# WPCLab/OpenSeg3D

Measured on AMD Instinct MI355X. Metric: points/sec fwd+bwd, Waymo 1-sweep ~180k pts @0.1m voxel; logit parity, higher is better.
Workload: dtype f32 storage/accumulate, bf16x3 products; 1 GPU; waymo_one_sweep (BASELINE configs[1]): synthetic scene, 174633 pts/step/GPU, voxel [0.1, 0.1, 0.1], grid [1440, 1440, 64], fwd (attention dropout p=0.1, DropPath) + criterion (ohem_ce+lovasz on 3 heads) + bwd + SGD step; mode=fwdbwd, segmentor=segformer, voxels=108690, parallelism=dp1

## Files before the change

include/seg3d_hip.h:

```cpp
#ifndef SEG3D_HIP_H
#define SEG3D_HIP_H

#include <stddef.h>
#include <stdint.h>

#ifdef __cplusplus
extern "C" {
#endif

#define SEG3D_OK 0
#define SEG3D_EINVAL (-1)
#define SEG3D_EWORKSPACE (-2)
#define SEG3D_ELAUNCH (-3)

#define SEG3D_REDUCE_SUM 0
#define SEG3D_REDUCE_MEAN 1
#define SEG3D_REDUCE_MAX 2

int seg3d_abi_version(void);

const char* seg3d_last_error(void);

int seg3d_grid_size(const float* voxel_size, const float* range, int32_t* grid_xyz);

// ... 324 lines not shown

#define SEG3D_CRITERION_MAX_HEADS 4
#define SEG3D_CRITERION_CE 1
#define SEG3D_CRITERION_LOVASZ 2
#define SEG3D_CRITERION_STATS_STRIDE 68
typedef struct {
    const float* logits;
    const int64_t* labels;
    int64_t n;
    float weight;
} seg3d_criterion_head;
typedef struct {
    int32_t n_heads;
    seg3d_criterion_head heads[SEG3D_CRITERION_MAX_HEADS];
} seg3d_criterion_table;
size_t seg3d_criterion_workspace_bytes(const seg3d_criterion_table* heads, int32_t c, int32_t terms);
int seg3d_criterion_fwd(const seg3d_criterion_table* heads, int32_t c, int32_t terms, int64_t ignore_index,
                        float keep_thresh, float w_ce, float w_lovasz, float* lse, float* coef, float* stats, float* loss,
                        void* workspace, size_t workspace_bytes, void* stream);
int seg3d_criterion_bwd(const seg3d_criterion_table* heads, int32_t c, int32_t terms, float w_ce, float w_lovasz,
                        const float* lse, const float* coef, const float* stats, const float* grad_out,
                        float* const* dlogits, void* stream);

size_t seg3d_pointwise_loss_workspace_bytes(int64_t n);
int seg3d_focal_loss_fwd(const float* logits, const int64_t* labels, int64_t n, int32_t c, int64_t ignore_index, float gamma,
                         float alpha, const float* class_weight, int32_t reduction, float* stats, void* workspace,
                         size_t workspace_bytes, void* stream);
int seg3d_focal_loss_bwd(const float* logits, const int64_t* labels, const float* stats, const float* grad_out, int64_t n,
                         int32_t c, int64_t ignore_index, float gamma, float alpha, const float* class_weight,
                         int32_t reduction, float* dlogits, void* stream);

int seg3d_dice_loss_fwd(const float* logits, const int64_t* labels, int64_t n, int32_t c, int64_t ignore_index, float smooth,
                        float exponent, const float* class_weight, float loss_weight, float avg_factor, float* loss,
                        void* workspace, size_t workspace_bytes, void* stream);
int seg3d_dice_loss_bwd(const float* logits, const int64_t* labels, const float* grad_out, int64_t n, int32_t c,
                        int64_t ignore_index, float smooth, float exponent, const float* class_weight, float loss_weight,
                        float avg_factor, float* dlogits, void* stream);

#define SEG3D_CE_SELECT_MEAN_WEIGHTED 0
#define SEG3D_CE_SELECT_MEAN_ALL 1
#define SEG3D_CE_SELECT_THRESH 2
#define SEG3D_CE_SELECT_RATIO 3
size_t seg3d_ce_select_workspace_bytes(int64_t n);
int seg3d_ce_select_fwd(const float* logits, const int64_t* labels, int64_t n, int32_t c, int64_t ignore_index,
                        const float* class_weight, int32_t mode, float keep_thresh, double keep_ratio, float* lse,
                        float* stats, void* workspace, size_t workspace_bytes, void* stream);
// ... 187 lines not shown
```

openseg3d_amd/_lib.py:

```python
import ctypes
import os
import re

_HERE = os.path.dirname(os.path.abspath(__file__))
LIB_PATH = os.path.join(_HERE, "csrc", "libseg3d_hip.so")
HEADER_PATH = os.path.join(os.path.dirname(_HERE), "include", "seg3d_hip.h")

OK, EINVAL, EWORKSPACE, ELAUNCH = 0, -1, -2, -3
REDUCE_SUM, REDUCE_MEAN, REDUCE_MAX = 0, 1, 2
ABI_VERSION = 53

_p, _i32, _i64, _sz, _f = ctypes.c_void_p, ctypes.c_int32, ctypes.c_int64, ctypes.c_size_t, ctypes.c_float
_u64 = ctypes.c_uint64
_d = ctypes.c_double

SIGNATURES = {
    "seg3d_abi_version": (ctypes.c_int, []),
    "seg3d_last_error": (ctypes.c_char_p, []),
    "seg3d_grid_size": (ctypes.c_int, [_p, _p, _p]),
    "seg3d_voxelize_workspace_bytes": (_sz, [_i64]),
    "seg3d_voxelize_f32": (ctypes.c_int, [_p, _i64, _i32, _i32, _i32, _p, _p, _p, _p, _p, _p, _sz, _p]),
    "seg3d_voxelize_f64": (ctypes.c_int, [_p, _i64, _i32, _i32, _i32, _p, _p, _p, _p, _p, _p, _sz, _p]),
    "seg3d_voxelize_host_workspace_bytes": (_sz, [_i64]),
    "seg3d_voxelize_host_f32": (ctypes.c_int, [_p, _i64, _i32, _i32, _i32, _p, _p, _p, _p, _p, _p, _sz]),
    "seg3d_voxelize_host_f64": (ctypes.c_int, [_p, _i64, _i32, _i32, _i32, _p, _p, _p, _p, _p, _p, _sz]),
    "seg3d_cart2polar_f32": (ctypes.c_int, [_p, _i64, _i32, _i32, _p, _p]),
    "seg3d_cart2polar_f64": (ctypes.c_int, [_p, _i64, _i32, _i32, _p, _p]),
    "seg3d_group_index_workspace_bytes": (_sz, [_i64, _i64]),
    "seg3d_group_index": (ctypes.c_int, [_p, _i64, _i64, _p, _p, _p, _p, _sz, _p]),
    "seg3d_coord_hash_bytes": (_sz, [_i64]),
    "seg3d_coord_hash_build": (ctypes.c_int, [_p, _i64, _p, _p, _sz, _p]),
    "seg3d_rulebook_subm": (ctypes.c_int, [_p, _i64, _p, _p, _sz, _p, _p]),
    "seg3d_downsample_workspace_bytes": (_sz, [_i32, _p]),
# ... 55 lines not shown
    "seg3d_layernorm_bwd_workspace_bytes": (ctypes.c_size_t, [_i64, _i32]),
    "seg3d_layernorm_bwd": (ctypes.c_int, [_p, _p, _p, _p, _p, _p, _i64, _i32, _p, _p, _p, _p, ctypes.c_size_t, _p]),
    "seg3d_layernorm_bwd_partials": (ctypes.c_int, [_p, _p, _p, _p, _p, _p, _i64, _i32, _p, _p, ctypes.c_size_t, _p, _p]),
    "seg3d_batchnorm_workspace_bytes": (ctypes.c_size_t, [_i64, _i32]),
    "seg3d_colstats": (ctypes.c_int, [_p, _i64, _i32, _p, _p, ctypes.c_size_t, _p]),
    "seg3d_batchnorm_stats": (ctypes.c_int, [_p, _i64, _i32, _f, _p, _p, _f, _p, _p, _p, _p, ctypes.c_size_t, _p]),
    "seg3d_affine_act": (ctypes.c_int, [_p, _p, _p, _p, _i32, _i64, _i32, _p, _p]),
    "seg3d_gelu_fwd": (ctypes.c_int, [_p, _i64, _p, _p, _p]),
    "seg3d_batchnorm_bwd": (ctypes.c_int, [_p, _p, _p, _p, _p, _p, _i32, _i64, _i32, _p, _p, _p, _p, ctypes.c_size_t, _p]),
    "seg3d_batchnorm_bwd_reduce": (ctypes.c_int, [_p, _p, _p, _p, _p, _i32, _i64, _i32, _p, _p, ctypes.c_size_t, _p]),
    "seg3d_batchnorm_bwd_apply": (ctypes.c_int, [_p, _p, _p, _p, _p, _p, _p, _p, _i32, _i64, _i32, _p, _p, _p]),
    "seg3d_segment_reduce_fwd": (ctypes.c_int, [_p, _i32, _p, _p, _i64, _i32, _p, _p, _p]),
    "seg3d_segment_reduce_bwd": (ctypes.c_int, [_p, _i32, _p, _i64, _p, _p, _i64, _i32, _p, _p]),
    "seg3d_voxel_majority_labels": (ctypes.c_int, [_p, _p, _p, _i64, _i32, _p, _p]),
    "seg3d_cross_entropy_workspace_bytes": (ctypes.c_size_t, [_i64]),
    "seg3d_cross_entropy_fwd": (ctypes.c_int, [_p, _p, _i64, _i32, _i64, _f, _p, _p, _p, ctypes.c_size_t, _p]),
    "seg3d_cross_entropy_bwd": (ctypes.c_int, [_p, _p, _p, _p, _p, _i64, _i32, _p, _p]),
    "seg3d_lovasz_workspace_bytes": (ctypes.c_size_t, [_i64, _i32]),
    "seg3d_lovasz_softmax_fwd": (ctypes.c_int, [_p, _p, _i64, _i32, _i64, _i32, _p, _p, _p, _p, _p, ctypes.c_size_t, _p]),
    "seg3d_lovasz_softmax_bwd": (ctypes.c_int, [_p, _p, _p, _p, _i64, _i32, _p, _p]),
    "seg3d_criterion_workspace_bytes": (ctypes.c_size_t, [_p, _i32, _i32]),
    "seg3d_criterion_fwd": (ctypes.c_int, [_p, _i32, _i32, _i64, _f, _f, _f, _p, _p, _p, _p, _p, ctypes.c_size_t, _p]),
    "seg3d_criterion_bwd": (ctypes.c_int, [_p, _i32, _i32, _f, _f, _p, _p, _p, _p, _p, _p]),
    "seg3d_pointwise_loss_workspace_bytes": (ctypes.c_size_t, [_i64]),
    "seg3d_focal_loss_fwd": (ctypes.c_int, [_p, _p, _i64, _i32, _i64, _f, _f, _p, _i32, _p, _p, ctypes.c_size_t, _p]),
    "seg3d_focal_loss_bwd": (ctypes.c_int, [_p, _p, _p, _p, _i64, _i32, _i64, _f, _f, _p, _i32, _p, _p]),
    "seg3d_dice_loss_fwd": (ctypes.c_int, [_p, _p, _i64, _i32, _i64, _f, _f, _p, _f, _f, _p, _p, ctypes.c_size_t, _p]),
    "seg3d_dice_loss_bwd": (ctypes.c_int, [_p, _p, _p, _i64, _i32, _i64, _f, _f, _p, _f, _f, _p, _p]),
    "seg3d_ce_select_workspace_bytes": (ctypes.c_size_t, [_i64]),
    "seg3d_ce_select_fwd": (ctypes.c_int, [_p, _p, _i64, _i32, _i64, _p, _i32, _f, ctypes.c_double, _p, _p, _p,
                                           ctypes.c_size_t, _p]),
    "seg3d_ce_select_bwd": (ctypes.c_int, [_p, _p, _p, _p, _p, _p, _i64, _i32, _i32, _p, _p]),
    "seg3d_knn_level_workspace_bytes": (ctypes.c_size_t, [_i64]),
    "seg3d_knn_level_build": (ctypes.c_int, [_p, _i64, _p, _i32, _f, _p, _p, _p, _p, _p, _i64, _p, ctypes.c_size_t, _p]),
    "seg3d_parity_order": (ctypes.c_int, [_p, _i64, _p, _p, ctypes.c_size_t, _p]),
    "seg3d_knn_query_order": (ctypes.c_int, [_p, _i64, _p, _i32, _f, _p, _p, ctypes.c_size_t, _p]),
    "seg3d_knn_grid_query": (ctypes.c_int, [_p, _i32, _p, _p, _i64, _p, _p, _i32, _i32, _p, _p, _p]),
    "seg3d_knn_query": (ctypes.c_int, [_p, _i64, _p, _i64, _p, _p, _i32, _i32, _p, _p, _p]),
    "seg3d_furthest_sampling_workspace_bytes": (_sz, [_i64]),
    "seg3d_furthest_sampling": (ctypes.c_int, [_p, _i64, _p, _p, _p, _i32, _p, _p, _sz, _p]),
    "seg3d_furthest_sampling_host": (ctypes.c_int, [_p, _i64, _p, _p, _p, _i32, _p]),
    "seg3d_sector_angles": (ctypes.c_int, [_p, _i64, _p, _i32, _p, _p, _p]),
    "seg3d_sector_angles_host": (ctypes.c_int, [_p, _i64, _p, _i32, _p, _p]),
    "seg3d_sector_assign": (ctypes.c_int, [_p, _i64, _p, _i32, _p, _p, _p, _p]),
    "seg3d_sector_assign_host": (ctypes.c_int, [_p, _i64, _p, _i32, _p, _p, _p]),
    "seg3d_pointops_scratch_bytes": (_sz, [_i64, _i32, _i32]),
# ... 116 lines not shown
```

openseg3d_amd/csrc/criterion.hip:

```cpp
#include <rocprim/device/device_radix_sort.hpp>

#include "criterion_device.hpp"

namespace {

using crit::class_bits;
using crit::kChunk;
using crit::kMaxBlocks;
using crit::kMaxClasses;
using crit::kThreads;
using Key = unsigned long long;

constexpr int kMaxHeads = SEG3D_CRITERION_MAX_HEADS;
constexpr int kErrBits = 30;
constexpr uint32_t kErrMask = (1u << kErrBits) - 1u;
constexpr int kStatsStride = SEG3D_CRITERION_STATS_STRIDE;

struct Head {
    const float* x;
    const int64_t* y;
    float* dx;
    int n;
    int row0;
    int blk0, nblk;
    int bblk0;
    int nchunks;
    int chunk0;
    int64_t sorted0;
    float weight;
};

struct Heads {
    int nh;
    Head h[kMaxHeads];
};

struct Plan {
    Heads hd;
    int64_t rows, total;
    int row_blocks, bwd_blocks, pairs;
    int sort_bits;
    size_t sort_bytes;
};

__device__ __forceinline__ int head_of(const Heads& hd, int idx, int Head::*first) {
    int h = 0;
    for (int i = 1; i < hd.nh; ++i)
        if (idx >= hd.h[i].*first) h = i;
    return h;
}

__global__ __launch_bounds__(kThreads) void criterion_rows_kernel(Heads hd, int c, int terms, int64_t ignore_index,
                                                                  float keep_thresh, float* __restrict__ lse,
                                                                  float* __restrict__ ce_part ,
                                                                  Key* __restrict__ keys, uint32_t* __restrict__ vals) {
    const int hi = head_of(hd, (int)blockIdx.x, &Head::blk0);
    const Head& H = hd.h[hi];
    const int n = H.n;
    const int64_t in0 = (int64_t)H.row0 * c;
    const int blk = (int)blockIdx.x - H.blk0;
    const float* __restrict__ x = H.x;
    const int64_t* __restrict__ label = H.y;
    float loss = 0.f, cnt = 0.f;
    for (int64_t r = (int64_t)blk * kThreads + threadIdx.x; r < n; r += (int64_t)H.nblk * kThreads) {
        const float* __restrict__ row = x + r * c;
        float m, s;
        crit::softmax_stats(row, c, &m, &s);
        const int64_t y = label[r];
        if (terms & SEG3D_CRITERION_CE) {
            float l;
            const bool counted = crit::ce_row(row, c, y, ignore_index, keep_thresh, m, s, &l);
            lse[H.row0 + r] = counted ? l : INFINITY;
            if (counted) {
                loss += l - row[y];
                cnt += 1.f;
            }
        }
        if (terms & SEG3D_CRITERION_LOVASZ) {
            const bool valid = y != ignore_index;
            for (int j = 0; j < c; ++j) {
                const bool fg = valid && y == j;
                const int64_t at = in0 + (int64_t)j * n + r;
                keys[at] = ((Key)(hi * c + j) << kErrBits) | (crit::lovasz_err_bits(row, j, m, s, valid, fg) & kErrMask);
                vals[at] = (uint32_t)(H.row0 + r) | (fg ? 0x80000000u : 0u);
            }
        }
    }
    if (terms & SEG3D_CRITERION_CE) {
        crit::block_sum2(loss, cnt);
        if (threadIdx.x == 0) {
            ce_part[2 * blockIdx.x] = loss;
            ce_part[2 * blockIdx.x + 1] = cnt;
        }
    }
}

__global__ __launch_bounds__(kThreads) void criterion_count_kernel(Heads hd, const uint32_t* __restrict__ vals,
                                                                   int* __restrict__ chunk_cnt) {
    const Head& H = hd.h[head_of(hd, (int)blockIdx.x, &Head::chunk0)];
    const int local = (int)blockIdx.x - H.chunk0;
    const int seg = local / H.nchunks, chunk = local - seg * H.nchunks;
    const int t = crit::lovasz_chunk_count(vals + H.sorted0 + (int64_t)seg * H.n, H.n, chunk);
    if (threadIdx.x == 0) chunk_cnt[blockIdx.x] = t;
}

__global__ __launch_bounds__(64) void criterion_offsets_kernel(Heads hd, int c, const int* __restrict__ chunk_cnt,
                                                               int* __restrict__ chunk_off, int* __restrict__ total) {
    const int hi = (int)blockIdx.x / c, seg = (int)blockIdx.x - hi * c;
    const Head& H = hd.h[hi];
    const int at = H.chunk0 + seg * H.nchunks;
    const int t = crit::lovasz_segment_offsets(chunk_cnt + at, H.nchunks, chunk_off + at);
    if (threadIdx.x == 0) total[blockIdx.x] = t;
}

__global__ __launch_bounds__(kThreads) void criterion_grad_kernel(Heads hd, int c, const Key* __restrict__ keys,
                                                                  const uint32_t* __restrict__ vals,
                                                                  const int* __restrict__ chunk_off,
                                                                  const int* __restrict__ total, float* __restrict__ coef,
                                                                  float* __restrict__ part) {
    const int hi = head_of(hd, (int)blockIdx.x, &Head::chunk0);
    const Head& H = hd.h[hi];
    const int local = (int)blockIdx.x - H.chunk0;
    const int seg = local / H.nchunks, chunk = local - seg * H.nchunks;
    const int64_t seg0 = H.sorted0 + (int64_t)seg * H.n;
    const float t = crit::lovasz_chunk_grad(keys + seg0, vals + seg0, kErrMask, H.n, c, c - 1 - seg, chunk,
                                            chunk_off[blockIdx.x], total[hi * c + seg], coef);
    if (threadIdx.x == 0) part[blockIdx.x] = t;
}

__global__ __launch_bounds__(kThreads) void criterion_finalize_kernel(Heads hd, int c, int terms, float w_ce, float w_lovasz,
                                                                      const float* __restrict__ ce_part,
                                                                      const float* __restrict__ part,
                                                                      const int* __restrict__ total,
                                                                      float* __restrict__ stats, float* __restrict__ out) {
    for (int hi = 0; hi < hd.nh; ++hi) {
        const Head& H = hd.h[hi];
        float* st = stats + hi * kStatsStride;
        if (terms & SEG3D_CRITERION_CE) {
            float mean, count;
            crit::ce_mean(ce_part + 2 * H.blk0, H.nblk, &mean, &count);
            if (threadIdx.x == 0) {
                st[0] = mean;
                st[1] = count;
            }
            __syncthreads();
        }
        if (terms & SEG3D_CRITERION_LOVASZ) {
// ... 89 lines not shown
    Heads& hd = pl->hd;
    hd.nh = nh;
    int row0 = 0, blk0 = 0, bblk0 = 0, chunk0 = 0;
    const int tile = bwd_tile_rows(c, terms);
    for (int i = 0; i < nh; ++i) {
        Head& H = hd.h[i];
        const int64_t n = tab->heads[i].n;
        H.x = tab->heads[i].logits;
        H.y = tab->heads[i].labels;
        H.dx = nullptr;
        H.n = (int)n;
        H.weight = tab->heads[i].weight;
        H.row0 = row0;
        H.blk0 = blk0;
        H.nblk = (int)(ceil_div64(n, kThreads) > kMaxBlocks ? kMaxBlocks : ceil_div64(n, kThreads));
        H.bblk0 = bblk0;
        H.nchunks = (int)ceil_div64(n, kChunk);
        H.chunk0 = chunk0;
        row0 += (int)n;
        blk0 += H.nblk;
        bblk0 += (int)ceil_div64(n, tile);
        chunk0 += c * H.nchunks;
    }
    int64_t behind = 0;
    for (int i = nh - 1; i >= 0; --i) {
        hd.h[i].sorted0 = behind;
        behind += (int64_t)hd.h[i].n * c;
    }
    pl->rows = rows;
    pl->total = rows * c;
    pl->row_blocks = blk0;
    pl->bwd_blocks = bblk0;
    pl->pairs = chunk0;
    pl->sort_bits = kErrBits + class_bits(nh * c);
    pl->sort_bytes = 0;
    return SEG3D_OK;
}

int plan_sort_scratch(int terms, Plan* pl) {
    if (!(terms & SEG3D_CRITERION_LOVASZ) || pl->total == 0) return SEG3D_OK;
    rocprim::double_buffer<Key> k(nullptr, nullptr);
    rocprim::double_buffer<uint32_t> v(nullptr, nullptr);
    size_t bytes = 0;
    if (rocprim::radix_sort_pairs_desc(nullptr, bytes, k, v, (size_t)pl->total, 0u, (unsigned)pl->sort_bits) != hipSuccess)
        return SEG3D_ELAUNCH;
    pl->sort_bytes = bytes;
    return SEG3D_OK;
}

size_t fixed_bytes(const Plan& pl, int c, int terms) {
    size_t b = align_up((size_t)(pl.row_blocks > 0 ? pl.row_blocks : 1) * 2 * sizeof(float), 256);
    if (terms & SEG3D_CRITERION_LOVASZ) {
        const size_t t = (size_t)pl.total, cc = (size_t)pl.pairs;
        b += 2 * align_up(t * sizeof(Key), 256) + 2 * align_up(t * sizeof(uint32_t), 256) + 2 * align_up(cc * sizeof(int), 256) +
             align_up(cc * sizeof(float), 256) + align_up((size_t)pl.hd.nh * c * sizeof(int), 256);
    }
    return b + 256;
}

}

extern "C" size_t seg3d_criterion_workspace_bytes(const seg3d_criterion_table* heads, int32_t c, int32_t terms) {
    Plan pl;
    if (make_plan(heads, c, terms, &pl) != SEG3D_OK || plan_sort_scratch(terms, &pl) != SEG3D_OK) return 0;
    return fixed_bytes(pl, c, terms) + align_up(pl.sort_bytes, 256);
}

extern "C" int seg3d_criterion_fwd(const seg3d_criterion_table* heads, int32_t c, int32_t terms, int64_t ignore_index,
                                   float keep_thresh, float w_ce, float w_lovasz, float* lse, float* coef, float* stats,
// ... 9 lines not shown
    if (workspace_bytes < fixed_bytes(pl, c, terms) + align_up(pl.sort_bytes, 256)) return SEG3D_EWORKSPACE;
    hipStream_t st = as_stream(stream);
    WsCarver ws(workspace);
    float* ce_part = ws.take<float>((size_t)(pl.row_blocks > 0 ? pl.row_blocks : 1) * 2);
    Key *k0 = nullptr, *k1 = nullptr;
    uint32_t *v0 = nullptr, *v1 = nullptr;
    int *chunk_cnt = nullptr, *chunk_off = nullptr, *total = nullptr;
    float* part = nullptr;
    void* sort_tmp = nullptr;
    if (lov) {
        const size_t t = (size_t)pl.total, cc = (size_t)pl.pairs;
        k0 = ws.take<Key>(t);
        k1 = ws.take<Key>(t);
        v0 = ws.take<uint32_t>(t);
        v1 = ws.take<uint32_t>(t);
        chunk_cnt = ws.take<int>(cc);
        chunk_off = ws.take<int>(cc);
        part = ws.take<float>(cc);
        total = ws.take<int>((size_t)pl.hd.nh * c);
        sort_tmp = ws.take<char>(pl.sort_bytes);
    }
    const Key* ks = k0;
    const uint32_t* vs = v0;
    if (pl.row_blocks > 0) {
        hipLaunchKernelGGL(criterion_rows_kernel, dim3((unsigned)pl.row_blocks), dim3(kThreads), 0, st, pl.hd, c, terms,
                           ignore_index, keep_thresh, lse, ce_part, k0, v0);
        SEG3D_CHECK_LAUNCH();
    }
    if (lov) {
        if (pl.total > 0) {
            rocprim::double_buffer<Key> kb(k0, k1);
            rocprim::double_buffer<uint32_t> vb(v0, v1);
            size_t bytes = pl.sort_bytes;
            SEG3D_CHECK_HIP(rocprim::radix_sort_pairs_desc(sort_tmp, bytes, kb, vb, (size_t)pl.total, 0u,
                                                           (unsigned)pl.sort_bits, st));
            ks = kb.current();
            vs = vb.current();
            hipLaunchKernelGGL(criterion_count_kernel, dim3((unsigned)pl.pairs), dim3(kThreads), 0, st, pl.hd, vs, chunk_cnt);
            SEG3D_CHECK_LAUNCH();
        }
        hipLaunchKernelGGL(criterion_offsets_kernel, dim3((unsigned)(pl.hd.nh * c)), dim3(64), 0, st, pl.hd, c, chunk_cnt,
                           chunk_off, total);
        SEG3D_CHECK_LAUNCH();
        if (pl.total > 0) {
            hipLaunchKernelGGL(criterion_grad_kernel, dim3((unsigned)pl.pairs), dim3(kThreads), 0, st, pl.hd, c, ks, vs,
                               chunk_off, total, coef, part);
            SEG3D_CHECK_LAUNCH();
        }
    }
    hipLaunchKernelGGL(criterion_finalize_kernel, dim3(1), dim3(kThreads), 0, st, pl.hd, c, terms, w_ce, w_lovasz, ce_part,
                       part, total, stats, loss);
    SEG3D_CHECK_LAUNCH();
    return SEG3D_OK;
}

extern "C" int seg3d_criterion_bwd(const seg3d_criterion_table* heads, int32_t c, int32_t terms, float w_ce, float w_lovasz,
                                   const float* lse, const float* coef, const float* stats, const float* grad_out,
                                   float* const* dlogits, void* stream) {
    Plan pl;
    const int rc = make_plan(heads, c, terms, &pl);
    if (rc != SEG3D_OK) return rc;
    const bool ce = terms & SEG3D_CRITERION_CE, lov = terms & SEG3D_CRITERION_LOVASZ;
    if (!stats || !grad_out || !dlogits) return SEG3D_EINVAL;
    if (pl.rows == 0) return SEG3D_OK;
    if ((ce && !lse) || (lov && !coef)) return SEG3D_EINVAL;
    for (int i = 0; i < pl.hd.nh; ++i) {
        if (pl.hd.h[i].n > 0 && !dlogits[i]) return SEG3D_EINVAL;
        pl.hd.h[i].dx = dlogits[i];
    }
    const int tile = bwd_tile_rows(c, terms);
    const size_t lds = (size_t)(lov ? 2 : 1) * tile * (c | 1) * sizeof(float);
    hipLaunchKernelGGL(criterion_bwd_kernel, dim3((unsigned)pl.bwd_blocks), dim3(kThreads), lds, as_stream(stream), pl.hd, c,
                       terms, tile, w_ce, w_lovasz, lse, coef, stats, grad_out);
    SEG3D_CHECK_LAUNCH();
    return SEG3D_OK;
}
```

openseg3d_amd/csrc/criterion_device.hpp:

```cpp
#pragma once
#include "common.hpp"

namespace crit {

constexpr int kThreads = 256;
constexpr int kMaxBlocks = 1024;
constexpr int kItems = 8;
constexpr int kChunk = kThreads * kItems;
constexpr int kMaxClasses = 64;

__device__ __forceinline__ void softmax_stats(const float* __restrict__ row, int c, float* m_out, float* s_out) {
    float m = row[0];
    for (int j = 1; j < c; ++j) m = fmaxf(m, row[j]);
    float s = 0.f;
    for (int j = 0; j < c; ++j) s += expf(row[j] - m);
    *m_out = m;
    *s_out = s;
}

__device__ __forceinline__ bool ce_row(const float* __restrict__ row, int c, int64_t y, int64_t ignore_index,
                                       float keep_thresh, float m, float s, float* lse_out) {
    *lse_out = m + logf(s);
    bool counted = y != ignore_index && y >= 0 && y < c;
    if (counted && keep_thresh > 0.f) counted = expf(row[y] - m) / s < keep_thresh;
// ... 58 lines not shown
    if (threadIdx.x == 0)
        for (int w = 0; w < kThreads / 64; ++w) t += red[w];
    return t;
}

__device__ __forceinline__ int lovasz_segment_offsets(const int* __restrict__ chunk_cnt, int nchunks,
                                                      int* __restrict__ chunk_off) {
    const int lane = threadIdx.x;
    int carry = 0;
    for (int t0 = 0; t0 < nchunks; t0 += 64) {
        const int i = t0 + lane;
        const int v = i < nchunks ? chunk_cnt[i] : 0;
        int inc = v;
        for (int off = 1; off < 64; off <<= 1) {
            const int o = __shfl_up(inc, off, SEG3D_WAVE);
            if (lane >= off) inc += o;
        }
        if (i < nchunks) chunk_off[i] = carry + inc - v;
        carry += __shfl(inc, 63, SEG3D_WAVE);
    }
    return carry;
}

__device__ __forceinline__ float lovasz_chunk_grad(const unsigned long long* __restrict__ keys,
                                                   const uint32_t* __restrict__ vals, uint32_t err_mask, int n, int c,
                                                   int cls, int chunk, int chunk_before, int total,
                                                   float* __restrict__ coef ) {
    const int base = chunk * kChunk + threadIdx.x * kItems;
    uint32_t v[kItems];
    float err[kItems];
    int mine = 0;
    for (int j = 0; j < kItems; ++j) {
        const bool in = base + j < n;
        v[j] = in ? vals[base + j] : 0u;
        err[j] = in ? __uint_as_float((uint32_t)keys[base + j] & err_mask) : 0.f;
        mine += (int)(v[j] >> 31);
    }
    const int lane = threadIdx.x & 63, wave = threadIdx.x >> 6;
    int inc = mine;
    for (int off = 1; off < 64; off <<= 1) {
        const int o = __shfl_up(inc, off, SEG3D_WAVE);
        if (lane >= off) inc += o;
    }
    __shared__ int wsum[kThreads / 64];
    __shared__ float wdot[kThreads / 64];
    if (lane == 63) wsum[wave] = inc;
    __syncthreads();
// ... 77 lines not shown
```

openseg3d_amd/csrc/voxelize.hip:

```cpp
#include <cstdio>

#include "common.hpp"

namespace {

constexpr int kThreads = 256;

struct VoxParams {
    int32_t grid[3];
    int32_t row_stride, xyz_col, batch_col;
};

template <typename T>
struct VoxConst {
    T lo[3];
    T vs[3];
};

__device__ __forceinline__ float floor_t(float v) { return floorf(v); }
__device__ __forceinline__ double floor_t(double v) { return floor(v); }

template <typename T>
__global__ __launch_bounds__(kThreads) void vox_insert(const T* __restrict__ pts, int64_t n, VoxParams p,
                                                       VoxConst<T> c, HashView h, uint32_t* __restrict__ slot_of) {
// ... 227 lines not shown
            o[2] = cc[1];
            o[3] = cc[0];
            ++count;
        }
        point_voxel_ids[i] = vals[s];
    }
    *n_voxels = count;
    return SEG3D_OK;
}

}

extern "C" {

int seg3d_cart2polar_f32(const float* points, int64_t n_points, int32_t row_stride, int32_t xyz_col, float* out, void* stream) {
    return cart2polar_impl<float>(points, n_points, row_stride, xyz_col, out, stream);
}

int seg3d_cart2polar_f64(const double* points, int64_t n_points, int32_t row_stride, int32_t xyz_col, double* out,
                         void* stream) {
    return cart2polar_impl<double>(points, n_points, row_stride, xyz_col, out, stream);
}

int seg3d_abi_version(void) { return 53; }

namespace {
thread_local char g_last_error[320] = "";
}

const char* seg3d_last_error(void) { return g_last_error; }

int seg3d_grid_size(const float* voxel_size, const float* range, int32_t* grid_xyz) {
    if (!voxel_size || !range || !grid_xyz) return SEG3D_EINVAL;
    for (int j = 0; j < 3; ++j) {
        volatile float span = range[3 + j] - range[j];
        volatile float g = span / voxel_size[j];
        grid_xyz[j] = (int32_t)__builtin_rintf(g);
        if (grid_xyz[j] <= 0) return SEG3D_EINVAL;
    }
    return SEG3D_OK;
}

size_t seg3d_voxelize_workspace_bytes(int64_t n_points) { return ws_bytes(n_points < 0 ? 0 : n_points); }

int seg3d_voxelize_f32(const float* points, int64_t n_points, int32_t row_stride, int32_t xyz_col, int32_t batch_col,
                       const float* voxel_size, const float* range, int32_t* voxel_coords, int32_t* point_voxel_ids,
                       int32_t* n_voxels, void* workspace, size_t workspace_bytes, void* stream) {
// ... 37 lines not shown
```

openseg3d_amd/ops.py:

```python
import ctypes
import weakref
import os

import numpy as np
import torch

from . import _lib
from ._lib import REDUCE_MAX, REDUCE_MEAN, REDUCE_SUM

_F3 = ctypes.c_float * 3
_F6 = ctypes.c_float * 6
_I3 = ctypes.c_int32 * 3


def _need_gpu(*tensors):
    for t in tensors:
        if t is not None and not t.is_cuda:
            raise _lib.Seg3dError("openseg3d_amd ops run on the GPU only (no CPU fallback); got a CPU tensor")


def _ptr(t):
    return None if t is None else ctypes.c_void_p(t.data_ptr())


# ... 51 lines not shown
            if WGRAD_DEFER and _defer_join(self, [(w, gr) for w, gr in grads if gr is not None and w is not None]):
                return
            st = _DEFERRED.get(_state_key(self.device))
            jobs = (st["jobs"] if st is not None else []) + self.jobs
            if st is not None:
                st["jobs"] = []
            if jobs:
                self.side.wait_stream(self.main)
                _run_reduce_jobs(jobs, self.device, self.side)
            ev = torch.cuda.Event()
            ev.record(self.side)
            self.main.wait_event(ev)
        elif self.jobs:
            _run_reduce_jobs(self.jobs, self.device, None)
        self.keep = []
        self.jobs = []


WGRAD_DEFER = os.environ.get("SEG3D_WGRAD_DEFER", "1") != "0"
_DEFERRED = {}
_DEFER_PROBE = {"done": False, "ok": None}
_MAX_IDLE_STATES = 4
DEFER_COUNT = 0


def _graph_task_id():
    fn = getattr(torch._C, "_current_graph_task_id", None)
    return fn() if fn is not None else -1


def _state_key(device):
    return (_graph_task_id(), device.index if device.index is not None else torch.cuda.current_device())


def _new_state(task, device):
    return {"keep": [], "main": None, "side": None, "seen": set(), "twice": set(), "fix": [], "task": task, "jobs": [],
            "jobs_device": device, "alias": {}}


def _reset_deferred():
    for key in list(_DEFERRED):
        _finish_state(key)


def _finish_state(key):
    st = _DEFERRED.pop(key, None)
# ... 127 lines not shown
                or _foreign_hooks(base)):
            return False
    if st is None:
        key, st = _state_for(fk)
        try:
            torch.autograd.Variable._execution_engine.queue_callback(lambda key=key: _finish_state(key))
        except RuntimeError:
            _DEFERRED.pop(key, None)
            return False
    for base, (w, gr) in zip(bases, grads):
        st["seen"].add(base.data_ptr())
        if w is base:
            st["fix"].append((base, gr.detach()))
            st["alias"][id(base)] = st["fix"][-1][1]
        else:
            st["keep"].append(gr.detach())
    global DEFER_COUNT
    DEFER_COUNT += 1
    st["main"], st["side"] = fk.main, fk.side
    st["keep"].append(fk.keep)
    st["jobs"].extend(fk.jobs)
    fk.keep = []
    fk.jobs = []
    return True


def probe_deferred_join(device):
    global WGRAD_DEFER
    pr = _DEFER_PROBE
    if pr["done"] or not (WGRAD_STREAM and WGRAD_DEFER) or device.type != "cuda":
        return pr["ok"]
    pr["done"] = True
    if _process_group_exists() and not len(DEFER_OWNED):
        return None
    before = WGRAD_DEFER
    try:
        with torch.cuda.device(device), torch.enable_grad():
            gen = torch.Generator().manual_seed(11)
            m, c = 16384, 64
            x = torch.randn(m, c, generator=gen).to(device)
            g = torch.randn(m, c, generator=gen).to(device)
            w0 = [(torch.randn(c, c, generator=gen) / 8.0).to(device) for _ in range(2)]
            b0 = [(torch.randn(c, generator=gen) * 0.1).to(device) for _ in range(2)]

            def grads(defer):
                global WGRAD_DEFER
# ... 3060 lines not shown
```

Baseline: 4.294 million points/s.

## Replace rocprim radix sort in Lovasz criterion with custom segmented 30-bit sort

Replaces the global rocprim radix sort over 64-bit (segment|error) keys with a custom per-segment LSD radix sort on 32-bit error keys, using 4 passes of 8/8/7/7 bits. Keys, values and histograms live in the existing key buffers, and the segment order is reversed via an ascending flag. The aim is to cut sort passes and halve key traffic, at the cost of more hand-written kernels and stability or ordering risk. It also adds an opt-in wgrad flush threshold and a debug sort entry point.

Result: no change. 4.320 million points/s, median of 6 (+0.6%).

```diff
diff --git a/include/seg3d_hip.h b/include/seg3d_hip.h
--- a/include/seg3d_hip.h
+++ b/include/seg3d_hip.h
@@ -370,6 +370,12 @@
                         const float* lse, const float* coef, const float* stats, const float* grad_out,
                         float* const* dlogits, void* stream);
 
+int32_t seg3d_debug_segmented_sort_tile(void);
+size_t seg3d_debug_segmented_sort_workspace_bytes(const int64_t* seg_lengths, int32_t n_segments);
+int seg3d_debug_segmented_sort_desc(const uint32_t* keys, const uint32_t* vals, const int64_t* seg_lengths,
+                                    int32_t n_segments, uint32_t* keys_out, uint32_t* vals_out, void* workspace,
+                                    size_t workspace_bytes, void* stream);
+
 size_t seg3d_pointwise_loss_workspace_bytes(int64_t n);
 int seg3d_focal_loss_fwd(const float* logits, const int64_t* labels, int64_t n, int32_t c, int64_t ignore_index, float gamma,
                          float alpha, const float* class_weight, int32_t reduction, float* stats, void* workspace,
diff --git a/openseg3d_amd/_lib.py b/openseg3d_amd/_lib.py
--- a/openseg3d_amd/_lib.py
+++ b/openseg3d_amd/_lib.py
@@ -8,7 +8,7 @@
 
 OK, EINVAL, EWORKSPACE, ELAUNCH = 0, -1, -2, -3
 REDUCE_SUM, REDUCE_MEAN, REDUCE_MAX = 0, 1, 2
-ABI_VERSION = 53
+ABI_VERSION = 54
 
 _p, _i32, _i64, _sz, _f = ctypes.c_void_p, ctypes.c_int32, ctypes.c_int64, ctypes.c_size_t, ctypes.c_float
 _u64 = ctypes.c_uint64
@@ -110,6 +110,9 @@
     "seg3d_criterion_workspace_bytes": (ctypes.c_size_t, [_p, _i32, _i32]),
     "seg3d_criterion_fwd": (ctypes.c_int, [_p, _i32, _i32, _i64, _f, _f, _f, _p, _p, _p, _p, _p, ctypes.c_size_t, _p]),
     "seg3d_criterion_bwd": (ctypes.c_int, [_p, _i32, _i32, _f, _f, _p, _p, _p, _p, _p, _p]),
+    "seg3d_debug_segmented_sort_tile": (_i32, []),
+    "seg3d_debug_segmented_sort_workspace_bytes": (ctypes.c_size_t, [_p, _i32]),
+    "seg3d_debug_segmented_sort_desc": (ctypes.c_int, [_p, _p, _p, _i32, _p, _p, _p, ctypes.c_size_t, _p]),
     "seg3d_pointwise_loss_workspace_bytes": (ctypes.c_size_t, [_i64]),
     "seg3d_focal_loss_fwd": (ctypes.c_int, [_p, _p, _i64, _i32, _i64, _f, _f, _p, _i32, _p, _p, ctypes.c_size_t, _p]),
     "seg3d_focal_loss_bwd": (ctypes.c_int, [_p, _p, _p, _p, _i64, _i32, _i64, _f, _f, _p, _i32, _p, _p]),
diff --git a/openseg3d_amd/csrc/criterion.hip b/openseg3d_amd/csrc/criterion.hip
--- a/openseg3d_amd/csrc/criterion.hip
+++ b/openseg3d_amd/csrc/criterion.hip
@@ -1,6 +1,10 @@
 #include <rocprim/device/device_radix_sort.hpp>
 
+#include <cstdlib>
+#include <cstring>
+
 #include "criterion_device.hpp"
+#include "segmented_sort.hpp"
 
 namespace {
 
@@ -27,6 +31,7 @@
     int nchunks;
     int chunk0;
     int64_t sorted0;
+    int ascending;
     float weight;
 };
 
@@ -39,9 +44,19 @@
     Heads hd;
     int64_t rows, total;
     int row_blocks, bwd_blocks, pairs;
+    bool own_sort;
+    segsort::Segments sg;
     int sort_bits;
     size_t sort_bytes;
 };
+
+bool use_own_sort() {
+    static const bool own = [] {
+        const char* e = getenv("SEG3D_CRITERION_SORT");
+        return !(e && strcmp(e, "rocprim") == 0);
+    }();
+    return own;
+}
 
 __device__ __forceinline__ int head_of(const Heads& hd, int idx, int Head::*first) {
     int h = 0;
@@ -50,10 +65,11 @@
     return h;
 }
 
+template <typename K>
 __global__ __launch_bounds__(kThreads) void criterion_rows_kernel(Heads hd, int c, int terms, int64_t ignore_index,
                                                                   float keep_thresh, float* __restrict__ lse,
                                                                   float* __restrict__ ce_part ,
-                                                                  Key* __restrict__ keys, uint32_t* __restrict__ vals) {
+                                                                  K* __restrict__ keys, uint32_t* __restrict__ vals) {
     const int hi = head_of(hd, (int)blockIdx.x, &Head::blk0);
     const Head& H = hd.h[hi];
     const int n = H.n;
@@ -81,7 +97,9 @@
             for (int j = 0; j < c; ++j) {
                 const bool fg = valid && y == j;
                 const int64_t at = in0 + (int64_t)j * n + r;
-                keys[at] = ((Key)(hi * c + j) << kErrBits) | (crit::lovasz_err_bits(row, j, m, s, valid, fg) & kErrMask);
+                const uint32_t err = crit::lovasz_err_bits(row, j, m, s, valid, fg) & kErrMask;
+                if constexpr (sizeof(K) == sizeof(Key)) keys[at] = ((Key)(hi * c + j) << kErrBits) | err;
+                else keys[at] = err;
                 vals[at] = (uint32_t)(H.row0 + r) | (fg ? 0x80000000u : 0u);
             }
         }
@@ -95,12 +113,12 @@
     }
 }
 
-__global__ __launch_bounds__(kThreads) void criterion_count_kernel(Heads hd, const uint32_t* __restrict__ vals,
+__global__ __launch_bounds__(kThreads) void criterion_count_kernel(Heads hd, int c, const uint32_t* __restrict__ vals,
                                                                    int* __restrict__ chunk_cnt) {
     const Head& H = hd.h[head_of(hd, (int)blockIdx.x, &Head::chunk0)];
     const int local = (int)blockIdx.x - H.chunk0;
     const int seg = local / H.nchunks, chunk = local - seg * H.nchunks;
-    const int t = crit::lovasz_chunk_count(vals + H.sorted0 + (int64_t)seg * H.n, H.n, chunk);
+    const int t = crit::lovasz_chunk_count(vals + H.sorted0 + (int64_t)(H.ascending ? c - 1 - seg : seg) * H.n, H.n, chunk);
     if (threadIdx.x == 0) chunk_cnt[blockIdx.x] = t;
 }
 
@@ -113,7 +131,8 @@
     if (threadIdx.x == 0) total[blockIdx.x] = t;
 }
 
-__global__ __launch_bounds__(kThreads) void criterion_grad_kernel(Heads hd, int c, const Key* __restrict__ keys,
+template <typename K>
+__global__ __launch_bounds__(kThreads) void criterion_grad_kernel(Heads hd, int c, const K* __restrict__ keys,
                                                                   const uint32_t* __restrict__ vals,
                                                                   const int* __restrict__ chunk_off,
                                                                   const int* __restrict__ total, float* __restrict__ coef,
@@ -122,7 +141,7 @@
     const Head& H = hd.h[hi];
     const int local = (int)blockIdx.x - H.chunk0;
     const int seg = local / H.nchunks, chunk = local - seg * H.nchunks;
-    const int64_t seg0 = H.sorted0 + (int64_t)seg * H.n;
+    const int64_t seg0 = H.sorted0 + (int64_t)(H.ascending ? c - 1 - seg : seg) * H.n;
     const float t = crit::lovasz_chunk_grad(keys + seg0, vals + seg0, kErrMask, H.n, c, c - 1 - seg, chunk,
                                             chunk_off[blockIdx.x], total[hi * c + seg], coef);
     if (threadIdx.x == 0) part[blockIdx.x] = t;
@@ -258,11 +277,14 @@
         bblk0 += (int)ceil_div64(n, tile);
         chunk0 += c * H.nchunks;
     }
+    pl->own_sort = use_own_sort();
     int64_t behind = 0;
     for (int i = nh - 1; i >= 0; --i) {
-        hd.h[i].sorted0 = behind;
+        hd.h[i].ascending = pl->own_sort;
+        hd.h[i].sorted0 = pl->own_sort ? (int64_t)hd.h[i].row0 * c : behind;
         behind += (int64_t)hd.h[i].n * c;
     }
+    if (!segsort::make_segments(nh * c, [&](int s) { return (int64_t)hd.h[s / c].n; }, &pl->sg)) return SEG3D_EINVAL;
     pl->rows = rows;
     pl->total = rows * c;
     pl->row_blocks = blk0;
@@ -273,14 +295,21 @@
     return SEG3D_OK;
 }
 
+size_t hist_room(const Plan& pl) {
+    const size_t t = (size_t)pl.total;
+    return 2 * align_up(t * sizeof(Key), 256) - 2 * align_up(t * sizeof(uint32_t), 256);
+}
+
 int plan_sort_scratch(int terms, Plan* pl) {
     if (!(terms & SEG3D_CRITERION_LOVASZ) || pl->total == 0) return SEG3D_OK;
+    const size_t hist = segsort::hist_bytes(pl->sg);
+    const size_t own = hist > hist_room(*pl) ? hist : 0;
     rocprim::double_buffer<Key> k(nullptr, nullptr);
     rocprim::double_buffer<uint32_t> v(nullptr, nullptr);
     size_t bytes = 0;
     if (rocprim::radix_sort_pairs_desc(nullptr, bytes, k, v, (size_t)pl->total, 0u, (unsigned)pl->sort_bits) != hipSuccess)
         return SEG3D_ELAUNCH;
-    pl->sort_bytes = bytes;
+    pl->sort_bytes = bytes > own ? bytes : own;
     return SEG3D_OK;
 }
 
@@ -336,29 +365,50 @@
     }
     const Key* ks = k0;
     const uint32_t* vs = v0;
+    uint32_t* const e0 = reinterpret_cast<uint32_t*>(k0);
+    uint32_t* const e1 = lov ? reinterpret_cast<uint32_t*>(reinterpret_cast<char*>(k0) +
+                                                           align_up((size_t)pl.total * sizeof(uint32_t), 256))
+                             : nullptr;
     if (pl.row_blocks > 0) {
-        hipLaunchKernelGGL(criterion_rows_kernel, dim3((unsigned)pl.row_blocks), dim3(kThreads), 0, st, pl.hd, c, terms,
-                           ignore_index, keep_thresh, lse, ce_part, k0, v0);
+        if (pl.own_sort)
+            hipLaunchKernelGGL(criterion_rows_kernel<uint32_t>, dim3((unsigned)pl.row_blocks), dim3(kThreads), 0, st, pl.hd, c,
+                               terms, ignore_index, keep_thresh, lse, ce_part, e0, v0);
+        else
+            hipLaunchKernelGGL(criterion_rows_kernel<Key>, dim3((unsigned)pl.row_blocks), dim3(kThreads), 0, st, pl.hd, c,
+                               terms, ignore_index, keep_thresh, lse, ce_part, k0, v0);
         SEG3D_CHECK_LAUNCH();
     }
     if (lov) {
         if (pl.total > 0) {
-            rocprim::double_buffer<Key> kb(k0, k1);
-            rocprim::double_buffer<uint32_t> vb(v0, v1);
-            size_t bytes = pl.sort_bytes;
-            SEG3D_CHECK_HIP(rocprim::radix_sort_pairs_desc(sort_tmp, bytes, kb, vb, (size_t)pl.total, 0u,
-                                                           (unsigned)pl.sort_bits, st));
-            ks = kb.current();
-            vs = vb.current();
-            hipLaunchKernelGGL(criterion_count_kernel, dim3((unsigned)pl.pairs), dim3(kThreads), 0, st, pl.hd, vs, chunk_cnt);
+            if (pl.own_sort) {
+                const size_t hist = segsort::hist_bytes(pl.sg);
+                int* const hs = hist > hist_room(pl) ? static_cast<int*>(sort_tmp)
+                                                     : reinterpret_cast<int*>(reinterpret_cast<char*>(e1) +
+                                                                              align_up((size_t)pl.total * sizeof(uint32_t), 256));
+                segsort::sort_pairs_desc(pl.sg, e0, v0, e1, v1, e0, v0, hs, st);
+                SEG3D_CHECK_LAUNCH();
+            } else {
+                rocprim::double_buffer<Key> kb(k0, k1);
+                rocprim::double_buffer<uint32_t> vb(v0, v1);
+                size_t bytes = pl.sort_bytes;
+                SEG3D_CHECK_HIP(rocprim::radix_sort_pairs_desc(sort_tmp, bytes, kb, vb, (size_t)pl.total, 0u,
+                                                               (unsigned)pl.sort_bits, st));
+                ks = kb.current();
+                vs = vb.current();
+            }
+            hipLaunchKernelGGL(criterion_count_kernel, dim3((unsigned)pl.pairs), dim3(kThreads), 0, st, pl.hd, c, vs, chunk_cnt);
             SEG3D_CHECK_LAUNCH();
         }
         hipLaunchKernelGGL(criterion_offsets_kernel, dim3((unsigned)(pl.hd.nh * c)), dim3(64), 0, st, pl.hd, c, chunk_cnt,
                            chunk_off, total);
         SEG3D_CHECK_LAUNCH();
         if (pl.total > 0) {
-            hipLaunchKernelGGL(criterion_grad_kernel, dim3((unsigned)pl.pairs), dim3(kThreads), 0, st, pl.hd, c, ks, vs,
-                               chunk_off, total, coef, part);
+            if (pl.own_sort)
+                hipLaunchKernelGGL(criterion_grad_kernel<uint32_t>, dim3((unsigned)pl.pairs), dim3(kThreads), 0, st, pl.hd, c, e0,
+                                   vs, chunk_off, total, coef, part);
+            else
+                hipLaunchKernelGGL(criterion_grad_kernel<Key>, dim3((unsigned)pl.pairs), dim3(kThreads), 0, st, pl.hd, c, ks, vs,
+                                   chunk_off, total, coef, part);
             SEG3D_CHECK_LAUNCH();
         }
     }
@@ -389,3 +439,42 @@
     SEG3D_CHECK_LAUNCH();
     return SEG3D_OK;
 }
+
+namespace {
+
+int plan_debug_sort(const int64_t* seg_lengths, int32_t n_segments, segsort::Segments* sg, size_t* bytes) {
+    if (n_segments < 0 || n_segments > segsort::kMaxSegments || (n_segments > 0 && !seg_lengths)) return SEG3D_EINVAL;
+    if (!segsort::make_segments(n_segments, [&](int s) { return seg_lengths[s]; }, sg)) return SEG3D_EINVAL;
+    *bytes = 2 * align_up((size_t)segsort::total_of(*sg) * sizeof(uint32_t), 256) + align_up(segsort::hist_bytes(*sg), 256) + 256;
+    return SEG3D_OK;
+}
+
+}
+
+extern "C" int32_t seg3d_debug_segmented_sort_tile(void) { return segsort::kTile; }
+
+extern "C" size_t seg3d_debug_segmented_sort_workspace_bytes(const int64_t* seg_lengths, int32_t n_segments) {
+    segsort::Segments sg;
+    size_t bytes = 0;
+    return plan_debug_sort(seg_lengths, n_segments, &sg, &bytes) == SEG3D_OK ? bytes : 0;
+}
+
+extern "C" int seg3d_debug_segmented_sort_desc(const uint32_t* keys, const uint32_t* vals, const int64_t* seg_lengths,
+                                               int32_t n_segments, uint32_t* keys_out, uint32_t* vals_out, void* workspace,
+                                               size_t workspace_bytes, void* stream) {
+    segsort::Segments sg;
+    size_t bytes = 0;
+    const int rc = plan_debug_sort(seg_lengths, n_segments, &sg, &bytes);
+    if (rc != SEG3D_OK) return rc;
+    const size_t t = (size_t)segsort::total_of(sg);
+    if (t > 0 && (!keys || !vals || !keys_out || !vals_out)) return SEG3D_EINVAL;
+    if (!workspace || workspace_bytes < bytes) return SEG3D_EWORKSPACE;
+    if (t == 0) return SEG3D_OK;
+    WsCarver ws(workspace);
+    uint32_t* kt = ws.take<uint32_t>(t);
+    uint32_t* vt = ws.take<uint32_t>(t);
+    int* hist = ws.take<int>((size_t)segsort::tiles_of(sg) * segsort::kRadix);
+    segsort::sort_pairs_desc(sg, keys, vals, kt, vt, keys_out, vals_out, hist, as_stream(stream));
+    SEG3D_CHECK_LAUNCH();
+    return SEG3D_OK;
+}
diff --git a/openseg3d_amd/csrc/criterion_device.hpp b/openseg3d_amd/csrc/criterion_device.hpp
--- a/openseg3d_amd/csrc/criterion_device.hpp
+++ b/openseg3d_amd/csrc/criterion_device.hpp
@@ -104,7 +104,8 @@
     return carry;
 }
 
-__device__ __forceinline__ float lovasz_chunk_grad(const unsigned long long* __restrict__ keys,
+template <typename K>
+__device__ __forceinline__ float lovasz_chunk_grad(const K* __restrict__ keys,
                                                    const uint32_t* __restrict__ vals, uint32_t err_mask, int n, int c,
                                                    int cls, int chunk, int chunk_before, int total,
                                                    float* __restrict__ coef ) {
diff --git a/openseg3d_amd/csrc/segmented_sort.hpp b/openseg3d_amd/csrc/segmented_sort.hpp
--- /dev/null
+++ b/openseg3d_amd/csrc/segmented_sort.hpp
@@ -0,0 +1,236 @@
+#pragma once
+#include "common.hpp"
+
+namespace segsort {
+
+constexpr int kThreads = 256;
+constexpr int kWaves = kThreads / SEG3D_WAVE;
+constexpr int kItems = 16;
+constexpr int kTile = kThreads * kItems;
+constexpr int kRadix = 256;
+constexpr int kMaxSegments = 256;
+constexpr int kKeyBits = 30;
+constexpr int kPasses = 4;
+constexpr int kDigitBits[kPasses] = {8, 8, 7, 7};
+static_assert(kDigitBits[0] + kDigitBits[1] + kDigitBits[2] + kDigitBits[3] == kKeyBits, "the digits cover the key");
+
+struct Segments {
+    int n;
+    int start[kMaxSegments + 1];
+    int tile0[kMaxSegments + 1];
+};
+
+template <typename Len>
+inline bool make_segments(int n, Len len, Segments* sg) {
+    if (n < 0 || n > kMaxSegments) return false;
+    int64_t at = 0, tiles = 0;
+    for (int s = 0; s < n; ++s) {
+        const int64_t l = len(s);
+        if (l < 0 || l >= (int64_t)1 << 31) return false;
+        sg->start[s] = (int)at;
+        sg->tile0[s] = (int)tiles;
+        at += l;
+        tiles += ceil_div64(l, kTile);
+        if (at >= (int64_t)1 << 31) return false;
+    }
+    sg->n = n;
+    for (int s = n; s <= kMaxSegments; ++s) {
+        sg->start[s] = (int)at;
+        sg->tile0[s] = (int)tiles;
+    }
+    return true;
+}
+
+inline int64_t total_of(const Segments& sg) { return sg.start[sg.n]; }
+inline int tiles_of(const Segments& sg) { return sg.tile0[sg.n]; }
+inline size_t hist_bytes(const Segments& sg) { return (size_t)tiles_of(sg) * kRadix * sizeof(int); }
+
+__device__ __forceinline__ int segment_of_tile(const Segments& sg, int b) {
+    int lo = 0, hi = sg.n;
+    while (hi - lo > 1) {
+        const int mid = (lo + hi) >> 1;
+        if (sg.tile0[mid] <= b) lo = mid;
+        else hi = mid;
+    }
+    return lo;
+}
+
+template <int BITS>
+__global__ __launch_bounds__(kThreads) void segsort_hist_kernel(Segments sg, const uint32_t* __restrict__ keys, int shift,
+                                                                int* __restrict__ hist ) {
+    __shared__ int cnt[kRadix];
+    const int s = segment_of_tile(sg, (int)blockIdx.x);
+    const int first = sg.start[s] + ((int)blockIdx.x - sg.tile0[s]) * kTile;
+    const int m = sg.start[s + 1] - first < kTile ? sg.start[s + 1] - first : kTile;
+    const uint32_t* __restrict__ k = keys + first;
+    cnt[threadIdx.x] = 0;
+    uint32_t key[kItems];
+#pragma unroll
+    for (int i = 0; i < kItems; ++i) {
+        const int e = i * kThreads + (int)threadIdx.x;
+        key[i] = e < m ? k[e] : 0u;
+    }
+    __syncthreads();
+    uint32_t cur = 0;
+    int run = 0;
+#pragma unroll
+    for (int i = 0; i < kItems; ++i)
+        if (i * kThreads + (int)threadIdx.x < m) {
+            const uint32_t d = (key[i] >> shift) & ((1u << BITS) - 1u);
+            if (d != cur && run > 0) {
+                atomicAdd(&cnt[cur], run);
+                run = 0;
+            }
+            cur = d;
+            ++run;
+        }
+    if (run > 0) atomicAdd(&cnt[cur], run);
+    __syncthreads();
+    hist[(int64_t)blockIdx.x * kRadix + threadIdx.x] = cnt[threadIdx.x];
+}
+
+__device__ __forceinline__ void block_exclusive_scan2(int& a, int& b) {
+    __shared__ int wsum[2][kWaves];
+    const int lane = threadIdx.x & 63, wave = threadIdx.x >> 6;
+    int ia = a, ib = b;
+    for (int off = 1; off < 64; off <<= 1) {
+        const int oa = __shfl_up(ia, off, SEG3D_WAVE), ob = __shfl_up(ib, off, SEG3D_WAVE);
+        if (lane >= off) {
+            ia += oa;
+            ib += ob;
+        }
+    }
+    if (lane == 63) {
+        wsum[0][wave] = ia;
+        wsum[1][wave] = ib;
+    }
+    __syncthreads();
+    int ca = 0, cb = 0;
+    for (int w = 0; w < wave; ++w) {
+        ca += wsum[0][w];
+        cb += wsum[1][w];
+    }
+    a = ca + ia - a;
+    b = cb + ib - b;
+}
+
+template <int BITS>
+__global__ __launch_bounds__(kThreads) void segsort_scatter_kernel(Segments sg, const uint32_t* __restrict__ kin,
+                                                                   const uint32_t* __restrict__ vin,
+                                                                   uint32_t* __restrict__ kout, uint32_t* __restrict__ vout,
+                                                                   const int* __restrict__ hist, int shift) {
+    __shared__ uint32_t sk[kTile], sv[kTile];
+    __shared__ int wcnt[kWaves][kRadix];
+    __shared__ int lstart[kRadix];
+    __shared__ int dst[kRadix];
+    constexpr uint32_t kMask = (1u << BITS) - 1u;
+    const int tid = threadIdx.x, lane = tid & 63, wave = tid >> 6;
+    const int s = segment_of_tile(sg, (int)blockIdx.x);
+    const int seg0 = sg.start[s], seg_len = sg.start[s + 1] - seg0;
+    const int tile = (int)blockIdx.x - sg.tile0[s], ntiles = sg.tile0[s + 1] - sg.tile0[s];
+    const int first = seg0 + tile * kTile;
+    const int m = seg_len - tile * kTile < kTile ? seg_len - tile * kTile : kTile;
+
+#pragma unroll
+    for (int w = 0; w < kWaves; ++w) wcnt[w][tid] = 0;
+
+    uint32_t key[kItems], val[kItems];
+    const int wbase = wave * 64 * kItems + lane;
+#pragma unroll
+    for (int i = 0; i < kItems; ++i) {
+        const int e = wbase + i * 64;
+        key[i] = e < m ? kin[first + e] : 0u;
+        val[i] = e < m ? vin[first + e] : 0u;
+    }
+
+    const int D = kRadix - 1 - tid;
+    int seg_total = 0, tiles_before = 0;
+    {
+        const int* __restrict__ h = hist + (int64_t)sg.tile0[s] * kRadix + D;
+#pragma unroll 4
+        for (int t = 0; t < ntiles; ++t) {
+            const int c = h[(int64_t)t * kRadix];
+            seg_total += c;
+            tiles_before += t < tile ? c : 0;
+        }
+    }
+    __syncthreads();
+
+    int rank[kItems];
+    const uint64_t below = ((uint64_t)1 << lane) - 1u;
+#pragma unroll
+    for (int i = 0; i < kItems; ++i) {
+        const bool valid = wbase + i * 64 < m;
+        const uint32_t d = (key[i] >> shift) & kMask;
+        uint64_t peers = __ballot(valid);
+#pragma unroll
+        for (int b = 0; b < BITS; ++b) {
+            const bool bit = (d >> b) & 1u;
+            const uint64_t bal = __ballot(bit);
+            peers &= bit ? bal : ~bal;
+        }
+        const int in_front = __popcll(peers & below);
+        const int seen = valid ? wcnt[wave][d] : 0;
+        __builtin_amdgcn_wave_barrier();
+        if (valid && in_front == 0) wcnt[wave][d] = seen + __popcll(peers);
+        __builtin_amdgcn_wave_barrier();
+        rank[i] = seen + in_front;
+    }
+    __syncthreads();
+
+    int tile_cnt = 0;
+#pragma unroll
+    for (int w = 0; w < kWaves; ++w) {
+        const int c = wcnt[w][D];
+        wcnt[w][D] = tile_cnt;
+        tile_cnt += c;
+    }
+    int local = tile_cnt, global = seg_total;
+    block_exclusive_scan2(local, global);
+    lstart[D] = local;
+    dst[D] = seg0 + global + tiles_before - local;
+    __syncthreads();
+
+#pragma unroll
+    for (int i = 0; i < kItems; ++i)
+        if (wbase + i * 64 < m) {
+            const uint32_t d = (key[i] >> shift) & kMask;
+            const int p = lstart[d] + wcnt[wave][d] + rank[i];
+            sk[p] = key[i];
+            sv[p] = val[i];
+        }
+    __syncthreads();
+
+#pragma unroll
+    for (int i = 0; i < kItems; ++i) {
+        const int p = i * kThreads + tid;
+        if (p < m) {
+            const uint32_t k = sk[p];
+            const int o = dst[(k >> shift) & kMask] + p;
+            if ((unsigned)(o - seg0) < (unsigned)seg_len) {
+                kout[o] = k;
+                vout[o] = sv[p];
+            }
+        }
+    }
+}
+
+template <int BITS>
+inline void launch_pass(const Segments& sg, const uint32_t* kin, const uint32_t* vin, uint32_t* kout, uint32_t* vout, int* hist,
+                        int shift, hipStream_t st) {
+    const dim3 grid((unsigned)tiles_of(sg)), block(kThreads);
+    hipLaunchKernelGGL(segsort_hist_kernel<BITS>, grid, block, 0, st, sg, kin, shift, hist);
+    hipLaunchKernelGGL(segsort_scatter_kernel<BITS>, grid, block, 0, st, sg, kin, vin, kout, vout, hist, shift);
+}
+
+inline void sort_pairs_desc(const Segments& sg, const uint32_t* keys, const uint32_t* vals, uint32_t* keys_tmp,
+                            uint32_t* vals_tmp, uint32_t* keys_out, uint32_t* vals_out, int* hist, hipStream_t st) {
+    static_assert(kPasses == 4, "the buffer order below is written out for four passes");
+    if (tiles_of(sg) == 0) return;
+    launch_pass<kDigitBits[0]>(sg, keys, vals, keys_tmp, vals_tmp, hist, 0, st);
+    launch_pass<kDigitBits[1]>(sg, keys_tmp, vals_tmp, keys_out, vals_out, hist, kDigitBits[0], st);
+    launch_pass<kDigitBits[2]>(sg, keys_out, vals_out, keys_tmp, vals_tmp, hist, kDigitBits[0] + kDigitBits[1], st);
+    launch_pass<kDigitBits[3]>(sg, keys_tmp, vals_tmp, keys_out, vals_out, hist, kKeyBits - kDigitBits[3], st);
+}
+
+}
diff --git a/openseg3d_amd/csrc/voxelize.hip b/openseg3d_amd/csrc/voxelize.hip
--- a/openseg3d_amd/csrc/voxelize.hip
+++ b/openseg3d_amd/csrc/voxelize.hip
@@ -273,7 +273,7 @@
     return cart2polar_impl<double>(points, n_points, row_stride, xyz_col, out, stream);
 }
 
-int seg3d_abi_version(void) { return 53; }
+int seg3d_abi_version(void) { return 54; }
 
 namespace {
 thread_local char g_last_error[320] = "";
diff --git a/openseg3d_amd/ops.py b/openseg3d_amd/ops.py
--- a/openseg3d_amd/ops.py
+++ b/openseg3d_amd/ops.py
@@ -97,6 +97,8 @@
 _DEFER_PROBE = {"done": False, "ok": None}
 _MAX_IDLE_STATES = 4
 DEFER_COUNT = 0
+WGRAD_FLUSH_BYTES = int(float(os.environ.get("SEG3D_WGRAD_FLUSH_MB", "0")) * (1 << 20))
+FLUSH_COUNT = 0
 
 
 def _graph_task_id():
@@ -270,6 +272,13 @@
     st["jobs"].extend(fk.jobs)
     fk.keep = []
     fk.jobs = []
+    if WGRAD_FLUSH_BYTES > 0 and sum(job[1] * job[2] * 4 for job in st["jobs"]) > WGRAD_FLUSH_BYTES:
+        global FLUSH_COUNT
+        FLUSH_COUNT += 1
+        st["side"].wait_stream(st["main"])
+        _run_reduce_jobs(st["jobs"], st["jobs_device"], st["side"])
+        st["keep"].append(st["jobs"])
+        st["jobs"] = []
     return True
 
 
```
